# MDFahimAnjum/AliasFree-Diffusion-Models-PyTorch

Hardware: AMD Instinct MI355X
Metric: train_step_images_per_sec (higher is better)
Workload: dtype f32; 1 GPU; CIFAR-10 32x32x3 synthetic, UNet variant=3 (Config D), batch 256/GPU, T=1000, AdamW lr 3e-4, random-init weights (seed 42); global_batch=256, parallelism=dp1, hip_graph=True, launch_mode=lanes

## Files before the change

aliasfree-diffusion-models-pytorch_amd/csrc/attn_mfma.hip:

```cpp
#include "common.h"
#include "h2_common.h"

namespace afd {

using f32x16 = __attribute__((ext_vector_type(16))) float;
constexpr int kTK = 64;
constexpr float kLog2e = 1.4426950408889634f, kLn2 = 0.6931471805599453f;

__device__ __forceinline__ float xhalf(float v) { return __shfl_xor(v, 32, kWave); }
__device__ __forceinline__ int acc_row(int r, int half) { return (r & 3) + 8 * (r >> 2) + 4 * half; }

using f2 = __attribute__((ext_vector_type(2))) float;
template <int D>
__device__ __forceinline__ void load_row(const float* __restrict__ p, f2 (&v)[D / 2]) {
#pragma unroll
  for (int q = 0; q < D / 4; ++q) {
    const float4 a = reinterpret_cast<const float4*>(p)[q];
    v[2 * q] = (f2){a.x, a.y}; v[2 * q + 1] = (f2){a.z, a.w};
  }
}
template <int D>
__device__ __forceinline__ void axpy(f2 (&acc)[D / 2], float s, const f2 (&v)[D / 2]) {
  const f2 ss = {s, s};
#pragma unroll
  for (int i = 0; i < D / 2; ++i) acc[i] = __builtin_elementwise_fma(ss, v[i], acc[i]);
}

using bf8 = __attribute__((ext_vector_type(8))) __bf16;
using bf2 = __attribute__((ext_vector_type(2))) __bf16;
__device__ __forceinline__ void split3(float x, __bf16& a, __bf16& b, __bf16& c) {
  a = (__bf16)x; const float r = x - (float)a;
  b = (__bf16)r; const float r2 = r - (float)b;
  c = (__bf16)r2;
}
template <int D>
__device__ __forceinline__ void row_frags(const float (&x)[D], int half, bf8 (&f)[3]) {
  bf8 p1, p2, p3;
#pragma unroll
  for (int j = 0; j < 8; ++j) {
    __bf16 a, b, c;
    split3(D == 8 ? x[j] : (half ? x[(8 + j) % D] : x[j]), a, b, c);
    p1[j] = a; p2[j] = b; p3[j] = c;
  }
  if (D == 8) { f[0] = p1; f[1] = half ? p1 : p2; f[2] = half ? p3 : p2; }
  else { f[0] = p1; f[1] = p2; f[2] = p3; }
}
template <int D>
__device__ __forceinline__ void stage_pieces(uint32_t* __restrict__ P, int rr, int jp, float v0, float v1) {
  __bf16 a0, b0, c0, a1, b1, c1;
  split3(v0, a0, b0, c0); split3(v1, a1, b1, c1);
  const int rec = D == 8 ? rr : (jp >> 2) * kTK + rr, w = jp & 3, ps = (D / 8) * kTK;
  P[(0 * ps + rec) * 4 + w] = __builtin_bit_cast(uint32_t, (bf2){a0, a1});
  P[(1 * ps + rec) * 4 + w] = __builtin_bit_cast(uint32_t, (bf2){b0, b1});
  P[(2 * ps + rec) * 4 + w] = __builtin_bit_cast(uint32_t, (bf2){c0, c1});
}
template <int D>
__device__ __forceinline__ void load_frags(const uint32_t* __restrict__ P, int row, int half, bf8 (&a)[3]) {
  const bf8* p = reinterpret_cast<const bf8*>(P);
  if (D == 8) { a[0] = p[(half ? 1 : 0) * kTK + row]; a[1] = p[(half ? 2 : 0) * kTK + row]; a[2] = p[(half ? 0 : 1) * kTK + row]; }
  else {
#pragma unroll
    for (int m = 0; m < 3; ++m) a[m] = p[(m * 2 + half) * kTK + row];
  }
}
template <int D>
__device__ __forceinline__ f32x16 dotx3(const bf8 (&a)[3], const bf8 (&b)[3]) {
  f32x16 c;
#pragma unroll
  for (int r = 0; r < 16; ++r) c[r] = 0.f;
  if (D == 8) {
#pragma unroll
    for (int m = 0; m < 3; ++m) c = __builtin_amdgcn_mfma_f32_32x32x16_bf16(a[m], b[m], c, 0, 0, 0);
  } else {
    constexpr int TA[6] = {0, 1, 0, 2, 1, 0}, TB[6] = {0, 0, 1, 0, 1, 2};
#pragma unroll
    for (int m = 0; m < 6; ++m) c = __builtin_amdgcn_mfma_f32_32x32x16_bf16(a[TA[m]], b[TB[m]], c, 0, 0, 0);
  }
  return c;
}

template <int D>
__device__ __forceinline__ f32x16 dotx3c(const bf8 (&a)[3], const bf8 (&b)[3], f32x16 c) {
  static_assert(D == 8, "dotx3c: head dim 8");
#pragma unroll
  for (int m = 0; m < 3; ++m) c = __builtin_amdgcn_mfma_f32_32x32x16_bf16(a[m], b[m], c, 0, 0, 0);
  return c;
}

template <int D>
__global__ __launch_bounds__(256, 2) void attn_fwd_mfma(const float* __restrict__ qkv, float* __restrict__ o,
                                                      float* __restrict__ lse, int heads, int L, float scale) {
  __shared__ __attribute__((aligned(16))) uint32_t Kp[3 * (D / 8) * kTK * 4];
  __shared__ __attribute__((aligned(16))) float Vr[kTK * D];
  const int b = blockIdx.z, h = blockIdx.y, C = heads * D;
  const int lane = threadIdx.x & 63, wv = threadIdx.x >> 6, half = lane >> 5, l31 = lane & 31;
  const float* qp = qkv + ((long)b * 3 * C + h * D) * L;
  const float* kp = qp + (long)C * L;
  const float* vp = kp + (long)C * L;
  const int q0 = blockIdx.x * 256 + wv * 64;
  bf8 bq[2][3];
#pragma unroll
  for (int j = 0; j < 2; ++j) {
    float x[D];
#pragma unroll
    for (int d = 0; d < D; ++d) x[d] = qp[(long)d * L + q0 + j * 32 + l31] * (scale * kLog2e);
    row_frags<D>(x, half, bq[j]);
  }
  float m[2] = {-INFINITY, -INFINITY}, l[2] = {0.f, 0.f};
  f2 oa[2][D / 2];
#pragma unroll
  for (int j = 0; j < 2; ++j)
#pragma unroll
    for (int i = 0; i < D / 2; ++i) oa[j][i] = (f2){0.f, 0.f};

  constexpr int NP = D / 8;
  const int jp0 = threadIdx.x >> 6, rr = threadIdx.x & 63;
  float kreg[NP][2], vreg[NP][2];
  auto fetch = [&](int k0) {
#pragma unroll
    for (int e = 0; e < NP; ++e)
#pragma unroll
      for (int h = 0; h < 2; ++h) {
        kreg[e][h] = kp[(long)(2 * (jp0 + 4 * e) + h) * L + k0 + rr];
        vreg[e][h] = vp[(long)(2 * (jp0 + 4 * e) + h) * L + k0 + rr];
      }
  };
  fetch(0);
  for (int k0 = 0; k0 < L; k0 += kTK) {
    __syncthreads();
#pragma unroll
    for (int e = 0; e < NP; ++e) {
      const int jp = jp0 + 4 * e;
      stage_pieces<D>(Kp, rr, jp, kreg[e][0], kreg[e][1]);
      *reinterpret_cast<float2*>(Vr + rr * D + 2 * jp) = make_float2(vreg[e][0], vreg[e][1]);
    }
    __syncthreads();
    if (k0 + kTK < L) fetch(k0 + kTK);
#pragma unroll
    for (int kt = 0; kt < kTK / 32; ++kt) {
      bf8 ak[3];
      load_frags<D>(Kp, kt * 32 + l31, half, ak);
      f32x16 sc[2];
#pragma unroll
      for (int j = 0; j < 2; ++j) {
        sc[j] = dotx3<D>(ak, bq[j]);
        float mx = sc[j][0];
#pragma unroll
        for (int r = 1; r < 16; ++r) mx = fmaxf(mx, sc[j][r]);
        mx = fmaxf(mx, xhalf(mx));
        const float mn = fmaxf(m[j], mx);
        const float alpha = __builtin_amdgcn_exp2f(m[j] - mn);
        l[j] *= alpha;
#pragma unroll
        for (int i = 0; i < D / 2; ++i) oa[j][i] *= alpha;
        m[j] = mn;
      }
#pragma unroll
      for (int r = 0; r < 16; ++r) {
        f2 v[D / 2];
        load_row<D>(Vr + (kt * 32 + acc_row(r, half)) * D, v);
#pragma unroll
        for (int j = 0; j < 2; ++j) {
          const float p = __builtin_amdgcn_exp2f(sc[j][r] - m[j]);
          l[j] += p;
          axpy<D>(oa[j], p, v);
        }
      }
    }
  }
#pragma unroll
  for (int j = 0; j < 2; ++j) {
    const float lt = l[j] + xhalf(l[j]);
    const float inv = 1.0f / lt;
    const int qi = q0 + j * 32 + l31;
#pragma unroll
    for (int d = 0; d < D; ++d) {
      const float mine = oa[j][d >> 1][d & 1];
      const float t = mine + xhalf(mine);
      if (half == 0) o[((long)b * C + h * D + d) * L + qi] = t * inv;
    }
    if (half == 0) lse[((long)b * heads + h) * L + qi] = (m[j] + __builtin_amdgcn_logf(lt)) * kLn2;
  }
}

using h2v = __attribute__((ext_vector_type(2))) _Float16;
using u32x4 = __attribute__((ext_vector_type(4))) uint32_t;
__device__ __forceinline__ float opaque_neg1() {
  float v;
  asm volatile("s_mov_b32 %0, 0xbf800000" : "=s"(v));
  return v;
}
__device__ __forceinline__ void pv_split16(const f32x16& sc, float off, float neg1, h8 (&p1)[2], h8 (&p2)[2]) {
#pragma unroll
  for (int g = 0; g < 2; ++g) {
    u32x4 w1, w2;
#pragma unroll
    for (int q = 0; q < 4; ++q) {
      const float x0 = __builtin_amdgcn_exp2f(sc[8 * g + 2 * q] - off), x1 = __builtin_amdgcn_exp2f(sc[8 * g + 2 * q + 1] - off);
      const h2v a = __builtin_convertvector((f2){x0, x1}, h2v);
      const h2v c = __builtin_convertvector((f2){__builtin_fmaf((float)a[0], neg1, x0), __builtin_fmaf((float)a[1], neg1, x1)}, h2v);
      w1[q] = __builtin_bit_cast(uint32_t, a);
      w2[q] = __builtin_bit_cast(uint32_t, c);
    }
    p1[g] = __builtin_bit_cast(h8, w1);
    p2[g] = __builtin_bit_cast(h8, w2);
  }
}

template <int D>
__global__ __launch_bounds__(256, 2) void attn_fwd_pv(const float* __restrict__ qkv, float* __restrict__ o,
                                                    float* __restrict__ lse, int heads, int L, float scale) {
  static_assert(D == 8, "attn_fwd_pv: head dim 8");
  __shared__ __attribute__((aligned(16))) uint32_t Kp[3 * kTK * 4];
  __shared__ __attribute__((aligned(16))) _Float16 Va[2 * 2 * 2 * 32 * 8];
  __shared__ float wmax[4];
  const int b = blockIdx.z, h = blockIdx.y, C = heads * D;
  const int lane = threadIdx.x & 63, wv = threadIdx.x >> 6, half = lane >> 5, l31 = lane & 31;
  const float* qp = qkv + ((long)b * 3 * C + h * D) * L;
  const float* kp = qp + (long)C * L;
  const float* vp = kp + (long)C * L;
  const int q0 = blockIdx.x * 256 + wv * 64;
  bf8 bq[2][3];
#pragma unroll
  for (int j = 0; j < 2; ++j) {
    float x[D];
#pragma unroll
    for (int d = 0; d < D; ++d) x[d] = qp[(long)d * L + q0 + j * 32 + l31] * (scale * kLog2e);
    row_frags<D>(x, half, bq[j]);
  }
  for (int i = threadIdx.x; i < 2 * 2 * 2 * 16 * 8; i += 256) {
    const int rec = i >> 3, m = 16 + (rec & 15), blk = rec >> 4;
    Va[(blk * 32 + m) * 8 + (i & 7)] = (m == 16 || m == 20) ? (_Float16)1.0f : (_Float16)0.0f;
  }
  float m[2] = {-INFINITY, -INFINITY};
  f32x16 acc[2];
#pragma unroll
  for (int j = 0; j < 2; ++j)
#pragma unroll
    for (int r = 0; r < 16; ++r) acc[j][r] = 0.f;
  float sv = __uint_as_float(kH2ScaleCapBits);
  const float neg1 = opaque_neg1();

  const int jp0 = threadIdx.x >> 6, rr = threadIdx.x & 63;
  const int rho = rr & 31, vh = (rho >> 2) & 1, vr = (rho & 3) + 4 * (rho >> 3);
  const int vbase = ((((rr >> 5) * 2 + (vr >> 3)) * 2 + vh) * 32) * 8 + (vr & 7);
  float kreg[2], vreg[2];
  auto fetch = [&](int k0) {
#pragma unroll
    for (int hh = 0; hh < 2; ++hh) {
      kreg[hh] = kp[(long)(2 * jp0 + hh) * L + k0 + rr];
      vreg[hh] = vp[(long)(2 * jp0 + hh) * L + k0 + rr];
    }
  };
  fetch(0);
  for (int k0 = 0; k0 < L; k0 += kTK) {
    {
      const float mv = wave_amax(fmaxf(fabsf(vreg[0]), fabsf(vreg[1])));
      if (lane == 0) wmax[wv] = mv;
    }
    __syncthreads();
    {
      const float sn = fminf(sv, h2_scale_for(fmaxf(fmaxf(wmax[0], wmax[1]), fmaxf(wmax[2], wmax[3]))));
      if (sn != sv) {
        const float f = sn * h2_inv_pow2(sv);
#pragma unroll
        for (int j = 0; j < 2; ++j)
#pragma unroll
          for (int r = 0; r < 8; ++r) acc[j][r] *= f;
        sv = sn;
      }
    }
    stage_pieces<D>(Kp, rr, jp0, kreg[0], kreg[1]);
#pragma unroll
    for (int hh = 0; hh < 2; ++hh) {
      _Float16 a, c;
      h2_split(vreg[hh], sv, a, c);
      Va[vbase + (2 * jp0 + hh) * 8] = a;
      Va[vbase + (2 * jp0 + hh + 8) * 8] = c;
    }
    __syncthreads();
    if (k0 + kTK < L) fetch(k0 + kTK);
#pragma unroll
    for (int kt = 0; kt < kTK / 32; ++kt) {
      bf8 ak[3];
      load_frags<D>(Kp, kt * 32 + l31, half, ak);
      const h8* va = reinterpret_cast<const h8*>(Va) + ((kt * 2) * 2 + half) * 32 + l31;
      const h8 av0 = va[0], av1 = va[2 * 32];
#pragma unroll
      for (int j = 0; j < 2; ++j) {
        f32x16 sc = dotx3<D>(ak, bq[j]);
        float mx = fmaxf(sc[0], sc[1]);
#pragma unroll
        for (int r = 2; r < 16; r += 2) mx = fmaxf(fmaxf(mx, sc[r]), sc[r + 1]);
        mx = fmaxf(mx, xhalf(mx));
        const float mn = fmaxf(m[j], mx);
        const float alpha = __builtin_amdgcn_exp2f(m[j] - mn);
        m[j] = mn;
#pragma unroll
        for (int r = 0; r < 9; ++r) acc[j][r] *= alpha;
        const float off = mn - 14.0f;
        h8 p1[2], p2[2];
        pv_split16(sc, off, neg1, p1, p2);
        __builtin_amdgcn_s_setprio(2);
        acc[j] = __builtin_amdgcn_mfma_f32_32x32x16_f16(av0, p1[0], acc[j], 0, 0, 0);
        acc[j] = __builtin_amdgcn_mfma_f32_32x32x16_f16(av1, p1[1], acc[j], 0, 0, 0);
        acc[j] = __builtin_amdgcn_mfma_f32_32x32x16_f16(av0, p2[0], acc[j], 0, 0, 0);
        acc[j] = __builtin_amdgcn_mfma_f32_32x32x16_f16(av1, p2[1], acc[j], 0, 0, 0);
        __builtin_amdgcn_s_setprio(0);
      }
    }
  }
  const float isv = h2_inv_pow2(sv);
#pragma unroll
  for (int j = 0; j < 2; ++j) {
    const float lt = acc[j][8];
    const float inv = isv / lt;
    const int qi = q0 + j * 32 + l31;
#pragma unroll
    for (int i = 0; i < 4; ++i)
      o[((long)b * C + h * D + 4 * half + i) * L + qi] = (acc[j][i] + acc[j][4 + i]) * inv;
    if (half == 0) lse[((long)b * heads + h) * L + qi] = (m[j] - 14.0f + __builtin_amdgcn_logf(lt)) * kLn2;
  }
}

template <int D, int TJ>
__global__ __launch_bounds__(256, 2) void attn_bwd_dq_mfma(const float* __restrict__ qkv, const float* __restrict__ o,
                                                         const float* __restrict__ d_o, const float* __restrict__ lse,
                                                         float* __restrict__ dqkv, float* __restrict__ delta_out,
                                                         int heads, int L, float scale) {
  __shared__ __attribute__((aligned(16))) uint32_t Kp[3 * (D / 8) * kTK * 4];
  __shared__ __attribute__((aligned(16))) uint32_t Vp[3 * (D / 8) * kTK * 4];
  __shared__ __attribute__((aligned(16))) float Kr[kTK * D];
  const int b = blockIdx.z, h = blockIdx.y, C = heads * D;
  const int lane = threadIdx.x & 63, wv = threadIdx.x >> 6, half = lane >> 5, l31 = lane & 31;
  const float* qp = qkv + ((long)b * 3 * C + h * D) * L;
  const float* kp = qp + (long)C * L;
  const float* vp = kp + (long)C * L;
  const long ob = ((long)b * C + h * D) * L;
  const int q0 = blockIdx.x * (128 * TJ) + wv * (32 * TJ);
  bf8 bq[TJ][3], bg[TJ][3];
  float lsq[TJ], dlt[TJ];
  f2 dq[TJ][D / 2];
#pragma unroll
  for (int j = 0; j < TJ; ++j) {
    const int qi = q0 + j * 32 + l31;
    float dpart = 0.f, xq[D], xg[D];
#pragma unroll
    for (int d = 0; d < D; ++d) {
      xq[d] = qp[(long)d * L + qi] * (scale * kLog2e);
      xg[d] = d_o[ob + (long)d * L + qi];
      dpart = fmaf(xg[d], o[ob + (long)d * L + qi], dpart);
    }
    row_frags<D>(xq, half, bq[j]);
    row_frags<D>(xg, half, bg[j]);
    dlt[j] = dpart;
    lsq[j] = lse[((long)b * heads + h) * L + qi] * kLog2e;
    if (half == 0) delta_out[((long)b * heads + h) * L + qi] = dlt[j];
#pragma unroll
    for (int i = 0; i < D / 2; ++i) dq[j][i] = (f2){0.f, 0.f};
  }
  constexpr int NP = D / 8;
  const int jp0 = threadIdx.x >> 6, rr = threadIdx.x & 63;
  float kreg[NP][2], vreg[NP][2];
  auto fetch = [&](int k0) {
#pragma unroll
    for (int e = 0; e < NP; ++e)
#pragma unroll
      for (int h = 0; h < 2; ++h) {
        kreg[e][h] = kp[(long)(2 * (jp0 + 4 * e) + h) * L + k0 + rr];
        vreg[e][h] = vp[(long)(2 * (jp0 + 4 * e) + h) * L + k0 + rr];
      }
  };
  fetch(0);
  for (int k0 = 0; k0 < L; k0 += kTK) {
    __syncthreads();
#pragma unroll
    for (int e = 0; e < NP; ++e) {
      const int jp = jp0 + 4 * e;
      stage_pieces<D>(Kp, rr, jp, kreg[e][0], kreg[e][1]);
      stage_pieces<D>(Vp, rr, jp, vreg[e][0], vreg[e][1]);
      *reinterpret_cast<float2*>(Kr + rr * D + 2 * jp) = make_float2(kreg[e][0], kreg[e][1]);
    }
    __syncthreads();
    if (k0 + kTK < L) fetch(k0 + kTK);
#pragma unroll
    for (int kt = 0; kt < kTK / 32; ++kt) {
      bf8 ak[3], av[3];
      load_frags<D>(Kp, kt * 32 + l31, half, ak);
      load_frags<D>(Vp, kt * 32 + l31, half, av);
      f32x16 sc[TJ], dp[TJ];
#pragma unroll
      for (int j = 0; j < TJ; ++j) {
        sc[j] = dotx3<D>(ak, bq[j]);
        dp[j] = dotx3<D>(av, bg[j]);
      }
#pragma unroll
      for (int r = 0; r < 16; ++r) {
        f2 kr[D / 2];
        load_row<D>(Kr + (kt * 32 + acc_row(r, half)) * D, kr);
#pragma unroll
        for (int j = 0; j < TJ; ++j) {
          const float ds = __builtin_amdgcn_exp2f(sc[j][r] - lsq[j]) * (dp[j][r] - dlt[j]);
          axpy<D>(dq[j], ds, kr);
        }
      }
    }
  }
#pragma unroll
  for (int j = 0; j < TJ; ++j) {
    const int qi = q0 + j * 32 + l31;
#pragma unroll
    for (int d = 0; d < D; ++d) {
      const float mine = dq[j][d >> 1][d & 1];
      const float t = mine + xhalf(mine);
      if (half == 0) dqkv[((long)b * 3 * C + h * D + d) * L + qi] = t * scale;
    }
  }
}

template <int D, int TJ>
__global__ __launch_bounds__(256, 2) void attn_bwd_dkv_mfma(const float* __restrict__ qkv, const float* __restrict__ d_o,
                                                          const float* __restrict__ lse, const float* __restrict__ delta,
                                                          float* __restrict__ dqkv, int heads, int L, float scale) {
  __shared__ __attribute__((aligned(16))) uint32_t Qp[3 * (D / 8) * kTK * 4];
  __shared__ __attribute__((aligned(16))) uint32_t Gp[3 * (D / 8) * kTK * 4];
  __shared__ __attribute__((aligned(16))) float Qr[kTK * D];
  __shared__ __attribute__((aligned(16))) float Gr[kTK * D];
  __shared__ float Ls[kTK];
  __shared__ float Ds[kTK];
  const int b = blockIdx.z, h = blockIdx.y, C = heads * D;
  const int lane = threadIdx.x & 63, wv = threadIdx.x >> 6, half = lane >> 5, l31 = lane & 31;
  const float* qp = qkv + ((long)b * 3 * C + h * D) * L;
  const float* kp = qp + (long)C * L;
  const float* vp = kp + (long)C * L;
  const float* gp = d_o + ((long)b * C + h * D) * L;
  const float* lp = lse + ((long)b * heads + h) * L;
  const float* dlp = delta + ((long)b * heads + h) * L;
  const int key0 = blockIdx.x * (128 * TJ) + wv * (32 * TJ);
  __shared__ bf8 Bf[4][TJ][2][3][64];
  f2 dk[TJ][D / 2], dv[TJ][D / 2];
#pragma unroll
  for (int j = 0; j < TJ; ++j) {
    float xk[D], xv[D];
#pragma unroll
    for (int d = 0; d < D; ++d) {
      xk[d] = kp[(long)d * L + key0 + j * 32 + l31] * (scale * kLog2e);
      xv[d] = vp[(long)d * L + key0 + j * 32 + l31];
    }
    bf8 t[3];
    row_frags<D>(xk, half, t);
#pragma unroll
    for (int m = 0; m < 3; ++m) Bf[wv][j][0][m][lane] = t[m];
    row_frags<D>(xv, half, t);
#pragma unroll
    for (int m = 0; m < 3; ++m) Bf[wv][j][1][m][lane] = t[m];
#pragma unroll
    for (int i = 0; i < D / 2; ++i) { dk[j][i] = (f2){0.f, 0.f}; dv[j][i] = (f2){0.f, 0.f}; }
  }
  constexpr int NP = D / 8;
  const int jp0 = threadIdx.x >> 6, rr = threadIdx.x & 63;
  float qreg[NP][2], greg[NP][2], lreg = 0.f, dreg = 0.f;
  auto fetch = [&](int t0) {
#pragma unroll
    for (int e = 0; e < NP; ++e)
#pragma unroll
      for (int hh = 0; hh < 2; ++hh) {
        qreg[e][hh] = qp[(long)(2 * (jp0 + 4 * e) + hh) * L + t0 + rr];
        greg[e][hh] = gp[(long)(2 * (jp0 + 4 * e) + hh) * L + t0 + rr];
      }
    if (threadIdx.x < kTK) { lreg = lp[t0 + threadIdx.x] * kLog2e; dreg = dlp[t0 + threadIdx.x]; }
  };
  fetch(0);
  for (int t0 = 0; t0 < L; t0 += kTK) {
    __syncthreads();
#pragma unroll
    for (int e = 0; e < NP; ++e) {
      const int jp = jp0 + 4 * e;
      stage_pieces<D>(Qp, rr, jp, qreg[e][0], qreg[e][1]);
      stage_pieces<D>(Gp, rr, jp, greg[e][0], greg[e][1]);
      *reinterpret_cast<float2*>(Qr + rr * D + 2 * jp) = make_float2(qreg[e][0], qreg[e][1]);
      *reinterpret_cast<float2*>(Gr + rr * D + 2 * jp) = make_float2(greg[e][0], greg[e][1]);
    }
    if (threadIdx.x < kTK) { Ls[threadIdx.x] = lreg; Ds[threadIdx.x] = dreg; }
    __syncthreads();
    if (t0 + kTK < L) fetch(t0 + kTK);
#pragma unroll
    for (int qt = 0; qt < kTK / 32; ++qt) {
      bf8 aq[3], ag[3];
      load_frags<D>(Qp, qt * 32 + l31, half, aq);
      load_frags<D>(Gp, qt * 32 + l31, half, ag);
      f32x16 sc[TJ], dp[TJ];
#pragma unroll
      for (int j = 0; j < TJ; ++j) {
        bf8 bkj[3], bvj[3];
#pragma unroll
        for (int m = 0; m < 3; ++m) { bkj[m] = Bf[wv][j][0][m][lane]; bvj[m] = Bf[wv][j][1][m][lane]; }
        sc[j] = dotx3<D>(aq, bkj);
        dp[j] = dotx3<D>(ag, bvj);
      }
#pragma unroll
      for (int r = 0; r < 16; ++r) {
        const int qr = qt * 32 + acc_row(r, half);
        f2 qrow[D / 2], grow[D / 2];
        load_row<D>(Qr + qr * D, qrow);
        load_row<D>(Gr + qr * D, grow);
        const float ls = Ls[qr], dl = Ds[qr];
#pragma unroll
        for (int j = 0; j < TJ; ++j) {
          const float p = __builtin_amdgcn_exp2f(sc[j][r] - ls);
          const float ds = p * (dp[j][r] - dl);
          axpy<D>(dv[j], p, grow);
          axpy<D>(dk[j], ds, qrow);
        }
        if ((r & 1) == 1) asm volatile("" ::: "memory");
      }
    }
  }
#pragma unroll
  for (int j = 0; j < TJ; ++j) {
    const int ki = key0 + j * 32 + l31;
#pragma unroll
    for (int d = 0; d < D; ++d) {
      const float mk = dk[j][d >> 1][d & 1], mv = dv[j][d >> 1][d & 1];
      const float tk = mk + xhalf(mk), tv = mv + xhalf(mv);
      if (half == 0) {
        dqkv[((long)b * 3 * C + C + h * D + d) * L + ki] = tk * scale;
        dqkv[((long)b * 3 * C + 2 * C + h * D + d) * L + ki] = tv;
      }
    }
  }
}

__global__ __launch_bounds__(256) void attn_delta_k(const float* __restrict__ o, const float* __restrict__ d_o, float* __restrict__ delta,
                                                    int heads, int D, int L, long total) {
  const long i = (long)blockIdx.x * 256 + threadIdx.x;
  if (i >= total) return;
  const int q = i % L; const long bh = i / L;
  const float* po = o + bh * D * L + q;
  const float* pg = d_o + bh * D * L + q;
  float s = 0.f;
  for (int d = 0; d < D; ++d) s = fmaf(pg[(long)d * L], po[(long)d * L], s);
  delta[i] = s;
}

__device__ __forceinline__ void split16(const f32x16& v, float neg1, h8 (&p1)[2], h8 (&p2)[2]) {
#pragma unroll
  for (int g = 0; g < 2; ++g) {
    u32x4 w1, w2;
#pragma unroll
    for (int q = 0; q < 4; ++q) {
      const float x0 = v[8 * g + 2 * q], x1 = v[8 * g + 2 * q + 1];
      const h2v a = __builtin_convertvector((f2){x0, x1}, h2v);
      const h2v c = __builtin_convertvector((f2){__builtin_fmaf((float)a[0], neg1, x0), __builtin_fmaf((float)a[1], neg1, x1)}, h2v);
      w1[q] = __builtin_bit_cast(uint32_t, a);
      w2[q] = __builtin_bit_cast(uint32_t, c);
    }
    p1[g] = __builtin_bit_cast(h8, w1);
    p2[g] = __builtin_bit_cast(h8, w2);
  }
}
__device__ __forceinline__ void pack16(const f32x16& v, h8 (&p)[2]) {
#pragma unroll
  for (int g = 0; g < 2; ++g) {
    u32x4 w;
#pragma unroll
    for (int q = 0; q < 4; ++q) w[q] = __builtin_bit_cast(uint32_t, __builtin_convertvector((f2){v[8 * g + 2 * q], v[8 * g + 2 * q + 1]}, h2v));
    p[g] = __builtin_bit_cast(h8, w);
  }
}

template <int D>
__global__ __launch_bounds__(256, 2) void attn_bwd_fused(const float* __restrict__ qkv, const float* __restrict__ d_o,
                                                       const float* __restrict__ lse, const float* __restrict__ delta,
                                                       float* __restrict__ dqkv, int heads, int L, float scale) {
  static_assert(D == 8, "attn_bwd_fused: head dim 8");
  constexpr int REC = 2 * 2 * 2 * 16;
  __shared__ __attribute__((aligned(16))) uint32_t Qp[3 * kTK * 4];
  __shared__ __attribute__((aligned(16))) uint32_t Gp[3 * kTK * 4];
  __shared__ __attribute__((aligned(16))) _Float16 QA[(REC + 1) * 8];
  __shared__ __attribute__((aligned(16))) _Float16 GA[(REC + 1) * 8];
  __shared__ __attribute__((aligned(16))) _Float16 KA[4 * (REC + 1) * 8];
  __shared__ __attribute__((aligned(16))) bf8 Bf[4][2][2][3][64];
  __shared__ __attribute__((aligned(16))) float Ls[kTK];
  __shared__ __attribute__((aligned(16))) float Ds[kTK];
  __shared__ float DQ[4][D][kTK];
  __shared__ float wmax[4][4];
  const int b = blockIdx.y, h = blockIdx.x, C = heads * D;
  const int lane = threadIdx.x & 63, wv = threadIdx.x >> 6, half = lane >> 5, l31 = lane & 31;
  const float* qp = qkv + ((long)b * 3 * C + h * D) * L;
  const float* kp = qp + (long)C * L;
  const float* vp = kp + (long)C * L;
  const float* gp = d_o + ((long)b * C + h * D) * L;
  const float* lp = lse + ((long)b * heads + h) * L;
  const float* dlp = delta + ((long)b * heads + h) * L;
  float* dqg = dqkv + ((long)b * 3 * C + h * D) * L;

  if (threadIdx.x < 8) { QA[REC * 8 + threadIdx.x] = (_Float16)0.f; GA[REC * 8 + threadIdx.x] = (_Float16)0.f; }
  if (threadIdx.x < 32) KA[(threadIdx.x >> 3) * (REC + 1) * 8 + REC * 8 + (threadIdx.x & 7)] = (_Float16)0.f;
  h8 perm[2];
#pragma unroll
  for (int g = 0; g < 2; ++g)
#pragma unroll
    for (int j = 0; j < 8; ++j) perm[g][j] = (l31 == acc_row(8 * g + j, half)) ? (_Float16)1.0f : (_Float16)0.0f;
  auto a_rec = [&](int t, int g) { return l31 < 16 ? ((t * 2 + g) * 2 + half) * 16 + l31 : REC; };
  const int jp0 = threadIdx.x >> 6, rr = threadIdx.x & 63;
  const int rho = rr & 31, sh = (rho >> 2) & 1, sr = (rho & 3) + 4 * (rho >> 3);
  const int sbase = ((((rr >> 5) * 2 + (sr >> 3)) * 2 + sh) * 16) * 8 + (sr & 7);

  float sq = __uint_as_float(kH2ScaleCapBits), sg = sq;
  const float neg1 = opaque_neg1();
  for (int kb = 0; kb < L; kb += 256) {
    const int key0 = kb + wv * 64;
    float v1 = 0.f, kmax = 0.f;
    float xk[2][D];
#pragma unroll
    for (int j = 0; j < 2; ++j) {
      float xs[D], xv[D];
      float n1 = 0.f;
#pragma unroll
      for (int d = 0; d < D; ++d) {
        xk[j][d] = kp[(long)d * L + key0 + j * 32 + l31];
        xs[d] = xk[j][d] * (scale * kLog2e);
        xv[d] = vp[(long)d * L + key0 + j * 32 + l31];
        n1 += fabsf(xv[d]); kmax = fmaxf(kmax, fabsf(xk[j][d]));
      }
      v1 = fmaxf(v1, n1);
      bf8 t[3];
      row_frags<D>(xs, half, t);
#pragma unroll
      for (int m = 0; m < 3; ++m) Bf[wv][j][0][m][lane] = t[m];
      row_frags<D>(xv, half, t);
#pragma unroll
      for (int m = 0; m < 3; ++m) Bf[wv][j][1][m][lane] = t[m];
    }
    v1 = wave_amax(v1);
    const float sk = h2_scale_for(wave_amax(kmax));
    if (half == 0) {
      const int kh = (l31 >> 2) & 1, kr = (l31 & 3) + 4 * (l31 >> 3);
#pragma unroll
      for (int j = 0; j < 2; ++j)
#pragma unroll
        for (int d = 0; d < D; ++d) {
          _Float16 a, c;
          h2_split(xk[j][d], sk, a, c);
          const int base = wv * (REC + 1) * 8 + (((j * 2 + (kr >> 3)) * 2 + kh) * 16) * 8 + (kr & 7);
          KA[base + d * 8] = a; KA[base + (d + 8) * 8] = c;
        }
    }
    f32x16 accV[2], accK[2];
#pragma unroll
    for (int j = 0; j < 2; ++j)
#pragma unroll
      for (int r = 0; r < 16; ++r) { accV[j][r] = 0.f; accK[j][r] = 0.f; }
    float sds = __uint_as_float(kH2ScaleCapBits);

    float qreg[2], greg[2], lreg = 0.f, dreg = 0.f;
    auto fetch = [&](int t0) {
#pragma unroll
      for (int hh = 0; hh < 2; ++hh) {
        qreg[hh] = qp[(long)(2 * jp0 + hh) * L + t0 + rr];
        greg[hh] = gp[(long)(2 * jp0 + hh) * L + t0 + rr];
      }
      if (threadIdx.x < kTK) { lreg = lp[t0 + threadIdx.x] * kLog2e; dreg = dlp[t0 + threadIdx.x]; }
    };
    auto dq_flush = [&](int t0) {
#pragma unroll
      for (int it = 0; it < 2; ++it) {
        const int d = threadIdx.x >> 5, q = (threadIdx.x & 31) + 32 * it;
        const float t = ((DQ[0][d][q] + DQ[1][d][q]) + DQ[2][d][q]) + DQ[3][d][q];
        float* dst = dqg + (long)d * L + t0 + q;
        *dst = kb == 0 ? t : *dst + t;
      }
    };
    fetch(0);
    for (int t0 = 0; t0 < L; t0 += kTK) {
      {
        const float mq = wave_amax(fmaxf(fabsf(qreg[0]), fabsf(qreg[1])));
        const float mg = wave_amax(fmaxf(fabsf(greg[0]), fabsf(greg[1])));
        const float md = wave_amax(fabsf(dreg));
        if (lane == 0) { wmax[0][wv] = mq; wmax[1][wv] = mg; wmax[2][wv] = md; wmax[3][wv] = v1; }
      }
      __syncthreads();
      const float mq = fmaxf(fmaxf(wmax[0][0], wmax[0][1]), fmaxf(wmax[0][2], wmax[0][3]));
      const float mg = fmaxf(fmaxf(wmax[1][0], wmax[1][1]), fmaxf(wmax[1][2], wmax[1][3]));
      const float md = fmaxf(fmaxf(wmax[2][0], wmax[2][1]), fmaxf(wmax[2][2], wmax[2][3]));
      const float v1g = fmaxf(fmaxf(wmax[3][0], wmax[3][1]), fmaxf(wmax[3][2], wmax[3][3]));
      {
        const float sqn = fminf(sq, h2_scale_for(mq)), sgn = fminf(sg, h2_scale_for(mg));
        const float sdn = fminf(sds, h2_scale_for(fmaf(v1g, mg, md)));
        const float sdc = fminf(sdn, h2_scale_for(mg) * 0x1p64f);
        const float fk = (sqn * h2_inv_pow2(sq)) * (sdc * h2_inv_pow2(sds)), fv = sgn * h2_inv_pow2(sg);
        if (fk != 1.0f || fv != 1.0f) {
#pragma unroll
          for (int j = 0; j < 2; ++j)
#pragma unroll
            for (int r = 0; r < 8; ++r) { accK[j][r] *= fk; accV[j][r] *= fv; }
        }
        sq = sqn; sg = sgn; sds = sdc;
      }
      const float cds = sds * (1.0f / 16384.0f);
      stage_pieces<D>(Qp, rr, jp0, qreg[0], qreg[1]);
      stage_pieces<D>(Gp, rr, jp0, greg[0] * cds, greg[1] * cds);
#pragma unroll
      for (int hh = 0; hh < 2; ++hh) {
        _Float16 a, c;
        h2_split(qreg[hh], sq, a, c);
        QA[sbase + (2 * jp0 + hh) * 8] = a; QA[sbase + (2 * jp0 + hh + 8) * 8] = c;
        h2_split(greg[hh], sg, a, c);
        GA[sbase + (2 * jp0 + hh) * 8] = a; GA[sbase + (2 * jp0 + hh + 8) * 8] = c;
      }
      if (threadIdx.x < kTK) Ls[threadIdx.x] = 14.0f - lreg;
      if (t0 > 0) dq_flush(t0 - kTK);
      if (threadIdx.x < kTK) Ds[threadIdx.x] = -dreg * cds;
      __syncthreads();
      if (t0 + kTK < L) fetch(t0 + kTK);
      const float udq = (scale * h2_inv_pow2(sds)) * h2_inv_pow2(sk);
#pragma unroll
      for (int qt = 0; qt < kTK / 32; ++qt) {
        const h8* qa = reinterpret_cast<const h8*>(QA);
        const h8* ga = reinterpret_cast<const h8*>(GA);
        const h8* ka = reinterpret_cast<const h8*>(KA) + wv * (REC + 1);
        f32x16 accQ;
#pragma unroll
        for (int r = 0; r < 16; ++r) accQ[r] = 0.f;
#pragma unroll
        for (int j = 0; j < 2; ++j) {
          f32x16 sc, dp;
#pragma unroll
          for (int r4 = 0; r4 < 4; ++r4) {
            const int qr = qt * 32 + 8 * r4 + 4 * half;
            const float4 ls = *reinterpret_cast<const float4*>(Ls + qr), dl = *reinterpret_cast<const float4*>(Ds + qr);
            sc[4 * r4] = ls.x; sc[4 * r4 + 1] = ls.y; sc[4 * r4 + 2] = ls.z; sc[4 * r4 + 3] = ls.w;
            dp[4 * r4] = dl.x; dp[4 * r4 + 1] = dl.y; dp[4 * r4 + 2] = dl.z; dp[4 * r4 + 3] = dl.w;
          }
          {
            bf8 aq[3], bkj[3];
            load_frags<D>(Qp, qt * 32 + l31, half, aq);
#pragma unroll
            for (int m = 0; m < 3; ++m) bkj[m] = Bf[wv][j][0][m][lane];
            sc = dotx3c<D>(aq, bkj, sc);
          }
          {
            bf8 ag[3], bvj[3];
            load_frags<D>(Gp, qt * 32 + l31, half, ag);
#pragma unroll
            for (int m = 0; m < 3; ++m) bvj[m] = Bf[wv][j][1][m][lane];
            dp = dotx3c<D>(ag, bvj, dp);
          }
#pragma unroll
          for (int r = 0; r < 16; ++r) {
            const float pv = __builtin_amdgcn_exp2f(sc[r]);
            sc[r] = pv;
            dp[r] *= pv;
          }
          __builtin_amdgcn_sched_barrier(0);
          h8 p1[2], p2[2];
          {
            split16(sc, neg1, p1, p2);
            const h8 ga0 = ga[a_rec(qt, 0)], ga1 = ga[a_rec(qt, 1)];
            __builtin_amdgcn_s_setprio(2);
            accV[j] = __builtin_amdgcn_mfma_f32_32x32x16_f16(ga0, p1[0], accV[j], 0, 0, 0);
            accV[j] = __builtin_amdgcn_mfma_f32_32x32x16_f16(ga1, p1[1], accV[j], 0, 0, 0);
            accV[j] = __builtin_amdgcn_mfma_f32_32x32x16_f16(ga0, p2[0], accV[j], 0, 0, 0);
            accV[j] = __builtin_amdgcn_mfma_f32_32x32x16_f16(ga1, p2[1], accV[j], 0, 0, 0);
          }
          __builtin_amdgcn_s_setprio(0);
          __builtin_amdgcn_sched_barrier(0);
          {
            split16(dp, neg1, p1, p2);
            const h8 qa0 = qa[a_rec(qt, 0)], qa1 = qa[a_rec(qt, 1)];
            __builtin_amdgcn_s_setprio(2);
            accK[j] = __builtin_amdgcn_mfma_f32_32x32x16_f16(qa0, p1[0], accK[j], 0, 0, 0);
            accK[j] = __builtin_amdgcn_mfma_f32_32x32x16_f16(qa1, p1[1], accK[j], 0, 0, 0);
            accK[j] = __builtin_amdgcn_mfma_f32_32x32x16_f16(qa0, p2[0], accK[j], 0, 0, 0);
            accK[j] = __builtin_amdgcn_mfma_f32_32x32x16_f16(qa1, p2[1], accK[j], 0, 0, 0);
          }
          __builtin_amdgcn_sched_barrier(0);
          const h8 ka0 = ka[a_rec(j, 0)], ka1 = ka[a_rec(j, 1)];
#pragma unroll
          for (int pc = 0; pc < 2; ++pc) {
            f32x16 t;
#pragma unroll
            for (int r = 0; r < 16; ++r) t[r] = 0.f;
            t = __builtin_amdgcn_mfma_f32_32x32x16_f16(pc ? p2[0] : p1[0], perm[0], t, 0, 0, 0);
            t = __builtin_amdgcn_mfma_f32_32x32x16_f16(pc ? p2[1] : p1[1], perm[1], t, 0, 0, 0);
            h8 e[2];
            pack16(t, e);
            accQ = __builtin_amdgcn_mfma_f32_32x32x16_f16(ka0, e[0], accQ, 0, 0, 0);
            accQ = __builtin_amdgcn_mfma_f32_32x32x16_f16(ka1, e[1], accQ, 0, 0, 0);
          }
          __builtin_amdgcn_s_setprio(0);
          __builtin_amdgcn_sched_barrier(0);
        }
#pragma unroll
        for (int i = 0; i < 4; ++i) DQ[wv][4 * half + i][qt * 32 + l31] = (accQ[i] + accQ[4 + i]) * udq;
      }
    }
    __syncthreads();
    dq_flush(L - kTK);
    {
      const float uk = (scale * h2_inv_pow2(sds)) * h2_inv_pow2(sq), uv = h2_inv_pow2(sg) * (1.0f / 16384.0f);
#pragma unroll
      for (int j = 0; j < 2; ++j) {
        const int ki = key0 + j * 32 + l31;
#pragma unroll
        for (int i = 0; i < 4; ++i) {
          dqkv[((long)b * 3 * C + C + h * D + 4 * half + i) * L + ki] = (accK[j][i] + accK[j][4 + i]) * uk;
          dqkv[((long)b * 3 * C + 2 * C + h * D + 4 * half + i) * L + ki] = (accV[j][i] + accV[j][4 + i]) * uv;
        }
      }
    }
    __syncthreads();
  }
}


bool attn_mfma8_ok(int d, int L) { return (d == 8 || d == 16) && L % 256 == 0; }
static int g_attn_pv = 1;
void attn_pv_set(int m) { g_attn_pv = m; }
void attn_mfma8_fwd(const float* qkv, float* o, float* lse, int B, int heads, int d, int L, float sc, hipStream_t s) {
  if (d == 8 && g_attn_pv) hipLaunchKernelGGL(attn_fwd_pv<8>, dim3(L / 256, heads, B), dim3(256), 0, s, qkv, o, lse, heads, L, sc);
  else if (d == 8) hipLaunchKernelGGL(attn_fwd_mfma<8>, dim3(L / 256, heads, B), dim3(256), 0, s, qkv, o, lse, heads, L, sc);
  else hipLaunchKernelGGL(attn_fwd_mfma<16>, dim3(L / 256, heads, B), dim3(256), 0, s, qkv, o, lse, heads, L, sc);
}
void attn_mfma8_bwd_dq(const float* qkv, const float* o, const float* d_o, const float* lse, float* dqkv, float* delta,
                       int B, int heads, int d, int L, float sc, hipStream_t s) {
  if (d == 8) hipLaunchKernelGGL((attn_bwd_dq_mfma<8, 2>), dim3(L / 256, heads, B), dim3(256), 0, s, qkv, o, d_o, lse, dqkv, delta, heads, L, sc);
  else hipLaunchKernelGGL((attn_bwd_dq_mfma<16, 1>), dim3(L / 128, heads, B), dim3(256), 0, s, qkv, o, d_o, lse, dqkv, delta, heads, L, sc);
}
bool attn_fused_bwd(const float* qkv, const float* o, const float* d_o, const float* lse, float* dqkv, float* delta, int B, int heads,
                    int d, int L, float sc, hipStream_t s) {
  if (d != 8 || !g_attn_pv || L % 256) return false;
  const long total = (long)B * heads * L;
  hipLaunchKernelGGL(attn_delta_k, dim3((unsigned)((total + 255) / 256)), dim3(256), 0, s, o, d_o, delta, heads, d, L, total);
  hipLaunchKernelGGL(attn_bwd_fused<8>, dim3(heads, B), dim3(256), 0, s, qkv, d_o, lse, delta, dqkv, heads, L, sc);
  return true;
}
void attn_mfma8_bwd_dkv(const float* qkv, const float* d_o, const float* lse, const float* delta, float* dqkv, int B, int heads, int L,
                        float sc, hipStream_t s) {
  hipLaunchKernelGGL((attn_bwd_dkv_mfma<8, 2>), dim3(L / 256, heads, B), dim3(256), 0, s, qkv, d_o, lse, delta, dqkv, heads, L, sc);
}

}
```

Before: 35940 images/s.

## Software-pipeline attention backward: interleave exp/split with MFMA stages across tiles

```diff
diff --git a/aliasfree-diffusion-models-pytorch_amd/csrc/attn_mfma.hip b/aliasfree-diffusion-models-pytorch_amd/csrc/attn_mfma.hip
--- a/aliasfree-diffusion-models-pytorch_amd/csrc/attn_mfma.hip
+++ b/aliasfree-diffusion-models-pytorch_amd/csrc/attn_mfma.hip
@@ -543,6 +543,13 @@
   delta[i] = s;
 }
 
+__device__ __forceinline__ void split_pair(float x0, float x1, float neg1, uint32_t& w1, uint32_t& w2) {
+  const h2v a = __builtin_convertvector((f2){x0, x1}, h2v);
+  const h2v c = __builtin_convertvector((f2){__builtin_fmaf((float)a[0], neg1, x0), __builtin_fmaf((float)a[1], neg1, x1)}, h2v);
+  w1 = __builtin_bit_cast(uint32_t, a);
+  w2 = __builtin_bit_cast(uint32_t, c);
+}
+struct BwdPieces { u32x4 v1[2], v2[2], k1[2], k2[2]; };
 __device__ __forceinline__ void split16(const f32x16& v, float neg1, h8 (&p1)[2], h8 (&p2)[2]) {
 #pragma unroll
   for (int g = 0; g < 2; ++g) {
@@ -574,12 +581,12 @@
                                                        const float* __restrict__ lse, const float* __restrict__ delta,
                                                        float* __restrict__ dqkv, int heads, int L, float scale) {
   static_assert(D == 8, "attn_bwd_fused: head dim 8");
-  constexpr int REC = 2 * 2 * 2 * 16;
+  constexpr int RECB = 2 * 16 + 1, REC = 4 * RECB;
   __shared__ __attribute__((aligned(16))) uint32_t Qp[3 * kTK * 4];
   __shared__ __attribute__((aligned(16))) uint32_t Gp[3 * kTK * 4];
-  __shared__ __attribute__((aligned(16))) _Float16 QA[(REC + 1) * 8];
-  __shared__ __attribute__((aligned(16))) _Float16 GA[(REC + 1) * 8];
-  __shared__ __attribute__((aligned(16))) _Float16 KA[4 * (REC + 1) * 8];
+  __shared__ __attribute__((aligned(16))) _Float16 QA[REC * 8];
+  __shared__ __attribute__((aligned(16))) _Float16 GA[REC * 8];
+  __shared__ __attribute__((aligned(16))) _Float16 KA[4 * REC * 8];
   __shared__ __attribute__((aligned(16))) bf8 Bf[4][2][2][3][64];
   __shared__ __attribute__((aligned(16))) float Ls[kTK];
   __shared__ __attribute__((aligned(16))) float Ds[kTK];
@@ -595,17 +602,21 @@
   const float* dlp = delta + ((long)b * heads + h) * L;
   float* dqg = dqkv + ((long)b * 3 * C + h * D) * L;
 
-  if (threadIdx.x < 8) { QA[REC * 8 + threadIdx.x] = (_Float16)0.f; GA[REC * 8 + threadIdx.x] = (_Float16)0.f; }
-  if (threadIdx.x < 32) KA[(threadIdx.x >> 3) * (REC + 1) * 8 + REC * 8 + (threadIdx.x & 7)] = (_Float16)0.f;
+  if (threadIdx.x < 32) {
+    const int z = ((threadIdx.x >> 3) * RECB + 32) * 8 + (threadIdx.x & 7);
+    QA[z] = (_Float16)0.f; GA[z] = (_Float16)0.f;
+  }
+  if (threadIdx.x < 128) KA[(threadIdx.x >> 5) * REC * 8 + (((threadIdx.x >> 3) & 3) * RECB + 32) * 8 + (threadIdx.x & 7)] = (_Float16)0.f;
   h8 perm[2];
 #pragma unroll
   for (int g = 0; g < 2; ++g)
 #pragma unroll
     for (int j = 0; j < 8; ++j) perm[g][j] = (l31 == acc_row(8 * g + j, half)) ? (_Float16)1.0f : (_Float16)0.0f;
-  auto a_rec = [&](int t, int g) { return l31 < 16 ? ((t * 2 + g) * 2 + half) * 16 + l31 : REC; };
+  const int a_lane = l31 < 16 ? half * 16 + l31 : 32;
+  auto a_rec = [&](int t, int g) { return (t * 2 + g) * RECB + a_lane; };
   const int jp0 = threadIdx.x >> 6, rr = threadIdx.x & 63;
   const int rho = rr & 31, sh = (rho >> 2) & 1, sr = (rho & 3) + 4 * (rho >> 3);
-  const int sbase = ((((rr >> 5) * 2 + (sr >> 3)) * 2 + sh) * 16) * 8 + (sr & 7);
+  const int sbase = (((rr >> 5) * 2 + (sr >> 3)) * RECB + sh * 16) * 8 + (sr & 7);
 
   float sq = __uint_as_float(kH2ScaleCapBits), sg = sq;
   const float neg1 = opaque_neg1();
@@ -643,7 +654,7 @@
         for (int d = 0; d < D; ++d) {
           _Float16 a, c;
           h2_split(xk[j][d], sk, a, c);
-          const int base = wv * (REC + 1) * 8 + (((j * 2 + (kr >> 3)) * 2 + kh) * 16) * 8 + (kr & 7);
+          const int base = wv * REC * 8 + ((j * 2 + (kr >> 3)) * RECB + kh * 16) * 8 + (kr & 7);
           KA[base + d * 8] = a; KA[base + (d + 8) * 8] = c;
         }
     }
@@ -655,20 +666,25 @@
     float sds = __uint_as_float(kH2ScaleCapBits);
 
     float qreg[2], greg[2], lreg = 0.f, dreg = 0.f;
+    const unsigned foff = 2 * jp0 * L + rr;
     auto fetch = [&](int t0) {
+      unsigned fo = foff, ft = threadIdx.x;
+      asm volatile("" : "+v"(fo), "+v"(ft));
 #pragma unroll
       for (int hh = 0; hh < 2; ++hh) {
-        qreg[hh] = qp[(long)(2 * jp0 + hh) * L + t0 + rr];
-        greg[hh] = gp[(long)(2 * jp0 + hh) * L + t0 + rr];
-      }
-      if (threadIdx.x < kTK) { lreg = lp[t0 + threadIdx.x] * kLog2e; dreg = dlp[t0 + threadIdx.x]; }
+        qreg[hh] = (qp + hh * L + t0)[fo];
+        greg[hh] = (gp + hh * L + t0)[fo];
+      }
+      if (threadIdx.x < kTK) { lreg = (lp + t0)[ft] * kLog2e; dreg = (dlp + t0)[ft]; }
     };
     auto dq_flush = [&](int t0) {
 #pragma unroll
       for (int it = 0; it < 2; ++it) {
         const int d = threadIdx.x >> 5, q = (threadIdx.x & 31) + 32 * it;
         const float t = ((DQ[0][d][q] + DQ[1][d][q]) + DQ[2][d][q]) + DQ[3][d][q];
-        float* dst = dqg + (long)d * L + t0 + q;
+        unsigned dq_o = d * L + q;
+        asm volatile("" : "+v"(dq_o));
+        float* dst = dqg + t0 + dq_o;
         *dst = kb == 0 ? t : *dst + t;
       }
     };
@@ -715,86 +731,107 @@
       __syncthreads();
       if (t0 + kTK < L) fetch(t0 + kTK);
       const float udq = (scale * h2_inv_pow2(sds)) * h2_inv_pow2(sk);
-#pragma unroll
-      for (int qt = 0; qt < kTK / 32; ++qt) {
-        const h8* qa = reinterpret_cast<const h8*>(QA);
-        const h8* ga = reinterpret_cast<const h8*>(GA);
-        const h8* ka = reinterpret_cast<const h8*>(KA) + wv * (REC + 1);
-        f32x16 accQ;
-#pragma unroll
-        for (int r = 0; r < 16; ++r) accQ[r] = 0.f;
-#pragma unroll
-        for (int j = 0; j < 2; ++j) {
-          f32x16 sc, dp;
-#pragma unroll
-          for (int r4 = 0; r4 < 4; ++r4) {
-            const int qr = qt * 32 + 8 * r4 + 4 * half;
-            const float4 ls = *reinterpret_cast<const float4*>(Ls + qr), dl = *reinterpret_cast<const float4*>(Ds + qr);
-            sc[4 * r4] = ls.x; sc[4 * r4 + 1] = ls.y; sc[4 * r4 + 2] = ls.z; sc[4 * r4 + 3] = ls.w;
-            dp[4 * r4] = dl.x; dp[4 * r4 + 1] = dl.y; dp[4 * r4 + 2] = dl.z; dp[4 * r4 + 3] = dl.w;
+      const h8* qa = reinterpret_cast<const h8*>(QA);
+      const h8* ga = reinterpret_cast<const h8*>(GA);
+      const h8* ka = reinterpret_cast<const h8*>(KA) + wv * REC;
+      auto phase_a = [&](int qt, int j, f32x16& sc, f32x16& dp) __attribute__((always_inline)) {
+#pragma unroll
+        for (int r4 = 0; r4 < 4; ++r4) {
+          const int qr = qt * 32 + 8 * r4 + 4 * half;
+          const float4 ls = *reinterpret_cast<const float4*>(Ls + qr), dl = *reinterpret_cast<const float4*>(Ds + qr);
+          sc[4 * r4] = ls.x; sc[4 * r4 + 1] = ls.y; sc[4 * r4 + 2] = ls.z; sc[4 * r4 + 3] = ls.w;
+          dp[4 * r4] = dl.x; dp[4 * r4 + 1] = dl.y; dp[4 * r4 + 2] = dl.z; dp[4 * r4 + 3] = dl.w;
+        }
+        {
+          bf8 aq[3], bkj[3];
+          load_frags<D>(Qp, qt * 32 + l31, half, aq);
+#pragma unroll
+          for (int m = 0; m < 3; ++m) bkj[m] = Bf[wv][j][0][m][lane];
+          sc = dotx3c<D>(aq, bkj, sc);
+        }
+        __builtin_amdgcn_sched_barrier(0);
+        {
+          bf8 ag[3], bvj[3];
+          load_frags<D>(Gp, qt * 32 + l31, half, ag);
+#pragma unroll
+          for (int m = 0; m < 3; ++m) bvj[m] = Bf[wv][j][1][m][lane];
+          dp = dotx3c<D>(ag, bvj, dp);
+        }
+      };
+      auto phase_b = [&](int q, const f32x16& sc, const f32x16& dp, BwdPieces& P) __attribute__((always_inline)) {
+        const float x0 = __builtin_amdgcn_exp2f(sc[2 * q]), x1 = __builtin_amdgcn_exp2f(sc[2 * q + 1]);
+        const float y0 = dp[2 * q] * x0, y1 = dp[2 * q + 1] * x1;
+        uint32_t w1, w2;
+        split_pair(x0, x1, neg1, w1, w2);
+        P.v1[q >> 2][q & 3] = w1; P.v2[q >> 2][q & 3] = w2;
+        split_pair(y0, y1, neg1, w1, w2);
+        P.k1[q >> 2][q & 3] = w1; P.k2[q >> 2][q & 3] = w2;
+      };
+      f32x16 accQ, tq;
+      h8 ga0, ga1, qa0, qa1, ka0, ka1;
+      auto phase_c = [&](int s, int qt, int j, const BwdPieces& P) __attribute__((always_inline)) {
+        if (s == 0) { ga0 = ga[a_rec(qt, 0)]; ga1 = ga[a_rec(qt, 1)]; }
+        if (s == 1) { qa0 = qa[a_rec(qt, 0)]; qa1 = qa[a_rec(qt, 1)]; }
+        if (s == 2) { ka0 = ka[a_rec(j, 0)]; ka1 = ka[a_rec(j, 1)]; }
+        if (s == 0 || s == 1) {
+          const u32x4* pv = s ? P.v2 : P.v1;
+          accV[j] = __builtin_amdgcn_mfma_f32_32x32x16_f16(ga0, __builtin_bit_cast(h8, pv[0]), accV[j], 0, 0, 0);
+          accV[j] = __builtin_amdgcn_mfma_f32_32x32x16_f16(ga1, __builtin_bit_cast(h8, pv[1]), accV[j], 0, 0, 0);
+        } else if (s == 2 || s == 5) {
+          const u32x4* pk = s == 5 ? P.k2 : P.k1;
+#pragma unroll
+          for (int r = 0; r < 16; ++r) tq[r] = 0.f;
+          tq = __builtin_amdgcn_mfma_f32_32x32x16_f16(__builtin_bit_cast(h8, pk[0]), perm[0], tq, 0, 0, 0);
+          tq = __builtin_amdgcn_mfma_f32_32x32x16_f16(__builtin_bit_cast(h8, pk[1]), perm[1], tq, 0, 0, 0);
+        } else if (s == 3 || s == 6) {
+          const u32x4* pk = s == 6 ? P.k2 : P.k1;
+          accK[j] = __builtin_amdgcn_mfma_f32_32x32x16_f16(qa0, __builtin_bit_cast(h8, pk[0]), accK[j], 0, 0, 0);
+          accK[j] = __builtin_amdgcn_mfma_f32_32x32x16_f16(qa1, __builtin_bit_cast(h8, pk[1]), accK[j], 0, 0, 0);
+        } else {
+          h8 e[2];
+          pack16(tq, e);
+          if (s == 4 && j == 0) {
+#pragma unroll
+            for (int r = 0; r < 16; ++r) accQ[r] = 0.f;
           }
-          {
-            bf8 aq[3], bkj[3];
-            load_frags<D>(Qp, qt * 32 + l31, half, aq);
-#pragma unroll
-            for (int m = 0; m < 3; ++m) bkj[m] = Bf[wv][j][0][m][lane];
-            sc = dotx3c<D>(aq, bkj, sc);
-          }
-          {
-            bf8 ag[3], bvj[3];
-            load_frags<D>(Gp, qt * 32 + l31, half, ag);
-#pragma unroll
-            for (int m = 0; m < 3; ++m) bvj[m] = Bf[wv][j][1][m][lane];
-            dp = dotx3c<D>(ag, bvj, dp);
-          }
-#pragma unroll
-          for (int r = 0; r < 16; ++r) {
-            const float pv = __builtin_amdgcn_exp2f(sc[r]);
-            sc[r] = pv;
-            dp[r] *= pv;
-          }
+          accQ = __builtin_amdgcn_mfma_f32_32x32x16_f16(ka0, e[0], accQ, 0, 0, 0);
+          accQ = __builtin_amdgcn_mfma_f32_32x32x16_f16(ka1, e[1], accQ, 0, 0, 0);
+        }
+      };
+      auto dq_out = [&](int qt) __attribute__((always_inline)) {
+#pragma unroll
+        for (int i = 0; i < 4; ++i) DQ[wv][4 * half + i][qt * 32 + l31] = (accQ[i] + accQ[4 + i]) * udq;
+      };
+      BwdPieces pcs[2];
+      f32x16 sc, dp;
+      __builtin_amdgcn_s_setprio(2);
+      phase_a(0, 0, sc, dp);
+      __builtin_amdgcn_s_setprio(0);
+      __builtin_amdgcn_sched_barrier(0);
+#pragma unroll
+      for (int q = 0; q < 8; ++q) phase_b(q, sc, dp, pcs[0]);
+      __builtin_amdgcn_sched_barrier(0);
+#pragma unroll
+      for (int i = 1; i < 4; ++i) {
+        phase_a(i >> 1, i & 1, sc, dp);
+        __builtin_amdgcn_sched_barrier(0);
+#pragma unroll
+        for (int s = 0; s < 8; ++s) {
+          phase_c(s, (i - 1) >> 1, (i - 1) & 1, pcs[(i - 1) & 1]);
           __builtin_amdgcn_sched_barrier(0);
-          h8 p1[2], p2[2];
-          {
-            split16(sc, neg1, p1, p2);
-            const h8 ga0 = ga[a_rec(qt, 0)], ga1 = ga[a_rec(qt, 1)];
-            __builtin_amdgcn_s_setprio(2);
-            accV[j] = __builtin_amdgcn_mfma_f32_32x32x16_f16(ga0, p1[0], accV[j], 0, 0, 0);
-            accV[j] = __builtin_amdgcn_mfma_f32_32x32x16_f16(ga1, p1[1], accV[j], 0, 0, 0);
-            accV[j] = __builtin_amdgcn_mfma_f32_32x32x16_f16(ga0, p2[0], accV[j], 0, 0, 0);
-            accV[j] = __builtin_amdgcn_mfma_f32_32x32x16_f16(ga1, p2[1], accV[j], 0, 0, 0);
-          }
-          __builtin_amdgcn_s_setprio(0);
+          phase_b(s, sc, dp, pcs[i & 1]);
           __builtin_amdgcn_sched_barrier(0);
-          {
-            split16(dp, neg1, p1, p2);
-            const h8 qa0 = qa[a_rec(qt, 0)], qa1 = qa[a_rec(qt, 1)];
-            __builtin_amdgcn_s_setprio(2);
-            accK[j] = __builtin_amdgcn_mfma_f32_32x32x16_f16(qa0, p1[0], accK[j], 0, 0, 0);
-            accK[j] = __builtin_amdgcn_mfma_f32_32x32x16_f16(qa1, p1[1], accK[j], 0, 0, 0);
-            accK[j] = __builtin_amdgcn_mfma_f32_32x32x16_f16(qa0, p2[0], accK[j], 0, 0, 0);
-            accK[j] = __builtin_amdgcn_mfma_f32_32x32x16_f16(qa1, p2[1], accK[j], 0, 0, 0);
-          }
-          __builtin_amdgcn_sched_barrier(0);
-          const h8 ka0 = ka[a_rec(j, 0)], ka1 = ka[a_rec(j, 1)];
-#pragma unroll
-          for (int pc = 0; pc < 2; ++pc) {
-            f32x16 t;
-#pragma unroll
-            for (int r = 0; r < 16; ++r) t[r] = 0.f;
-            t = __builtin_amdgcn_mfma_f32_32x32x16_f16(pc ? p2[0] : p1[0], perm[0], t, 0, 0, 0);
-            t = __builtin_amdgcn_mfma_f32_32x32x16_f16(pc ? p2[1] : p1[1], perm[1], t, 0, 0, 0);
-            h8 e[2];
-            pack16(t, e);
-            accQ = __builtin_amdgcn_mfma_f32_32x32x16_f16(ka0, e[0], accQ, 0, 0, 0);
-            accQ = __builtin_amdgcn_mfma_f32_32x32x16_f16(ka1, e[1], accQ, 0, 0, 0);
-          }
-          __builtin_amdgcn_s_setprio(0);
-          __builtin_amdgcn_sched_barrier(0);
-        }
-#pragma unroll
-        for (int i = 0; i < 4; ++i) DQ[wv][4 * half + i][qt * 32 + l31] = (accQ[i] + accQ[4 + i]) * udq;
-      }
+        }
+        if (i == 2) dq_out(0);
+      }
+      __builtin_amdgcn_s_setprio(2);
+#pragma unroll
+      for (int s = 0; s < 8; ++s) {
+        phase_c(s, 1, 1, pcs[1]);
+        __builtin_amdgcn_sched_barrier(0);
+      }
+      __builtin_amdgcn_s_setprio(0);
+      dq_out(1);
     }
     __syncthreads();
     dq_flush(L - kTK);
```

After: 36100 images/s, median of 6. No clear change (+0.4%).
